# aligirayhanozbay/poisson_CNN

Measured on AMD Instinct MI355X. Metric: grids/sec (fwd+bwd) at 1024^2, higher is better.
Workload: dtype f32; 1 GPU; c4: Homogeneous_Poisson_NN_Legacy(hpnn.json) full train step (fwd+bwd+loss+Adam), 8 x 1024x1024 Dirichlet grids per GPU; global_batch=8, parallelism=dp1, math=fp32, ranks_seen=1

## Files before the change

### include/pcnn.h

```cpp
#ifndef PCNN_H
#define PCNN_H
#include <stddef.h>
#include <stdint.h>
#ifdef __cplusplus
extern "C" {
#endif

typedef struct pcnn_handle_s* pcnn_handle;

enum { PCNN_PAD_CONSTANT = 0, PCNN_PAD_SYMMETRIC = 1, PCNN_PAD_REFLECT = 2 };
enum { PCNN_ACT_LINEAR = 0, PCNN_ACT_LEAKY_RELU = 1, PCNN_ACT_TANH = 2, PCNN_ACT_RELU = 3 };
enum { PCNN_POOL_AVERAGE = 0, PCNN_POOL_MAX = 1 };
enum { PCNN_RESIZE_NEAREST = 0, PCNN_RESIZE_BILINEAR = 1, PCNN_RESIZE_BICUBIC = 2,
       PCNN_RESIZE_BICUBIC_LEGACY_ALIGN_CORNERS = 3  };

int pcnn_create(int device, void* hip_stream, pcnn_handle* out);
int pcnn_destroy(pcnn_handle h);
int pcnn_set_stream(pcnn_handle h, void* hip_stream);
int pcnn_sync(pcnn_handle h);
const char* pcnn_last_error(pcnn_handle h);
int pcnn_version(void);
uint32_t pcnn_crc32c(const void* data, size_t n, uint32_t crc);

#define PCNN_UNIQUE_ID_BYTES 128
// ... 77 lines not shown
int pcnn_conv2d_epilogue_bwd_absmax(pcnn_handle h, int64_t npix, int C, const float* dy, int lddy, const float* a, int lda,
                                    const float* bn_scale, int act, float act_alpha, float* dz, int lddz, float* dbias,
                                    float* dsum_dy_a, float* dsum_dy, float* dz_absmax, void* workspace, size_t workspace_bytes);

int pcnn_pad_fold_bwd(pcnn_handle h, int N, int H, int W, int C, int pt, int pb, int pl, int pr, int pad_mode,
                      const float* gp, int ldgp, float* gx, int ldgx, int accumulate);
int pcnn_pad_fold_bwd_post_eligible(int C, int ldgp, int ld_add, const void* gp, const void* add_to, const pcnn_post_desc* post, int lddz, const void* dz);
int pcnn_pad_fold_bwd_post(pcnn_handle h, int N, int H, int W, int C, int pt, int pb, int pl, int pr, int pad_mode, const float* gp, int ldgp,
                           const float* add_to, int ld_add, const pcnn_post_desc* post, const float* bn_scale, float* dsum_dy_a, float* dsum_dy,
                           float* dz, int lddz, void* workspace, size_t workspace_bytes);

int pcnn_bn_fold(pcnn_handle h, int n, const float* gamma, const float* beta, const float* mean, const float* var, float eps,
                 float* scale, float* shift);
int pcnn_bn_fold_bwd(pcnn_handle h, int n, const float* s_dy_a, const float* s_dy, const float* mean, const float* var, float eps,
                     float* dgamma, float* dbeta);

int pcnn_channel_affine(pcnn_handle h, int64_t npix, int C, const float* x, int ldx, const float* scale, const float* shift,
                        const float* residual, int ld_res, float* y, int ldy);
int pcnn_bn_train_fwd(pcnn_handle h, int64_t npix, int C, const float* a, int lda, const float* gamma, const float* beta, float eps,
                      float momentum, float* moving_mean, float* moving_var, float* mean, float* inv_std, float* scale, float* scratch_2C,
                      const float* residual, int ld_res, float* y, int ldy, void* workspace, size_t workspace_bytes);
int pcnn_bn_train_bwd(pcnn_handle h, int64_t npix, int C, const float* dy, int lddy, const float* a, int lda, const float* scale,
                      const float* mean, const float* inv_std, float* dgamma, float* dbeta, float* scratch_4C, float* da, int ldda,
                      void* workspace, size_t workspace_bytes);

int pcnn_pool2d_fwd(pcnn_handle h, int kind, int N, int H, int W, int C, int f, const float* x, int ldx, float* y, int ldy);
int pcnn_pool2d_bwd(pcnn_handle h, int kind, int N, int H, int W, int C, int f, const float* x, int ldx,
                    const float* y, int ldy, const float* dy, int lddy, float* dx, int lddx, int accumulate);

int pcnn_deconv_fwd(pcnn_handle h, int N, int hc, int wc, int Cin, int H, int W, int Cout, int f, const float* x, int ldx,
                    const float* k, const float* bias, float alpha, float beta, float* y, int ldy);
int pcnn_deconv_bwd_data(pcnn_handle h, int N, int hc, int wc, int Cin, int H, int W, int Cout, int f, const float* dy, int lddy,
                         const float* k, float alpha, float* dx, int lddx);
size_t pcnn_deconv_wgrad_workspace(int N, int hc, int wc, int Cin, int Cout, int f);
int pcnn_deconv_bwd_filter(pcnn_handle h, int N, int hc, int wc, int Cin, int H, int W, int Cout, int f, const float* x, int ldx,
                           const float* dy, int lddy, float alpha, float* dk, float* dbias, void* workspace, size_t workspace_bytes);

typedef struct {
  int N, H, W, Cin, ldx;
  int Ho, Wo, Cout, ldy;
  int k;
  int act; float act_alpha;
  float dropout_rate; uint32_t dropout_seed; uint32_t dropout_layer;
  int ld_act_out;
  int accumulate;
} pcnn_wide_desc;
int pcnn_wide_conv2d_fwd(pcnn_handle h, const pcnn_wide_desc* d, const float* x, const float* w, const float* bias, float* y);
int pcnn_wide_conv2d_dgrad(pcnn_handle h, const pcnn_wide_desc* d, const float* dz, const float* wf, const float* act_out, float* dx);
size_t pcnn_wide_conv2d_wgrad_workspace(const pcnn_wide_desc* d);
int pcnn_wide_conv2d_wgrad(pcnn_handle h, const pcnn_wide_desc* d, const float* x, const float* dz, float* dw, float* dbias, void* workspace,
                           size_t workspace_bytes);
int pcnn_wide_deconv_fwd(pcnn_handle h, const pcnn_wide_desc* d, const float* x, const float* k, const float* bias, float* y);
int pcnn_wide_deconv_bwd_data(pcnn_handle h, const pcnn_wide_desc* d, const float* dz, const float* k, const float* act_out, float* dx);
size_t pcnn_wide_deconv_bwd_filter_workspace(const pcnn_wide_desc* d);
int pcnn_wide_deconv_bwd_filter(pcnn_handle h, const pcnn_wide_desc* d, const float* x, const float* dz, float* dk, void* workspace,
                                size_t workspace_bytes);

int pcnn_resize_tables(int method, int n_in, int n_out, int32_t* idx , float* wt );
int pcnn_resize_fwd(pcnn_handle h, int N, int hc, int wc, int C, int Ho, int Wo, const float* x, int ldx,
                    const int32_t* idx_y, const float* wt_y, const int32_t* idx_x, const float* wt_x,
                    float alpha, float beta, float* y, int ldy);
typedef struct pcnn_resize_src {
  const float* x; int hc, wc, ldx;
  const int32_t* idx_y; const float* wt_y; const int32_t* idx_x; const float* wt_x;
} pcnn_resize_src;
int pcnn_resize_fwd_multi_eligible(int N, int C, int Ho, int Wo, int nsrc, const pcnn_resize_src* src, const float* y, int ldy);
// ... 135 lines not shown
```

### poisson_cnn_amd/csrc/deconv_mfma.hip

```cpp
#include "pcnn_internal.h"

namespace {

struct DeconvParams {
  int N, hc, wc, Cin, H, W, Cout, f, py, px;
  const float* x; int ldx;
  const float* wp;
  const float* bias;
  float alpha, beta;
  float* y; int ldy;
  const float* dy; int lddy;
  float* dx; int lddx;
  float* partial;
  int tiles_x, S;
  float* dummy;
};

__global__ void pack_deconv_fwd_kernel(const float* __restrict__ k, float* __restrict__ wp, int taps, int Cin, int Cout, int ng) {
  const int64_t total = (int64_t)taps * ng * 2 * 32 * 4;
  for (int64_t i = (int64_t)blockIdx.x * blockDim.x + threadIdx.x; i < total; i += (int64_t)gridDim.x * blockDim.x) {
    const int j = i & 3; int64_t r = i >> 2; const int co = r & 31; r >>= 5; const int h = r & 1; r >>= 1; const int g = r % ng; const int tap = r / ng;
    const int ci = 8 * g + 4 * h + j;
    wp[i] = (ci < Cin && co < Cout) ? k[((int64_t)tap * Cout + co) * Cin + ci] : 0.f;
  }
// ... 227 lines not shown
  hipLaunchKernelGGL(pack_deconv_bwd_kernel, dim3((unsigned)std::min<int64_t>(pcnn_cdiv64(tot, 256), 1024)), dim3(256), 0, h->stream, k,
                     static_cast<float*>(h->scratch), f * f, Cin, Cout, ng);
  DeconvParams p{};
  p.N = N; p.hc = hc; p.wc = wc; p.Cin = Cin; p.H = H; p.W = W; p.Cout = Cout; p.f = f; p.py = (hc * f - H) / 2; p.px = (wc * f - W) / 2;
  p.dy = dy; p.lddy = lddy; p.wp = static_cast<const float*>(h->scratch); p.alpha = alpha; p.dx = dx; p.lddx = lddx;
  p.tiles_x = pcnn_cdiv(wc, 32);
  const int64_t groups = (int64_t)N * hc * p.tiles_x;
  hipLaunchKernelGGL(deconv_bwd_data_mfma_kernel, dim3((unsigned)groups), dim3(256), 0, h->stream, p);
  PCNN_CHECK_LAUNCH(h, "pcnn_deconv_bwd_data(mfma)");
  return 0;
}

int pcnn_deconv_bwd_filter_splits(int N, int hc, int f) {
  int S = 1024 / (f * f);
  const int rows4 = (N * hc + 3) / 4;
  if (S > rows4) S = rows4;
  if (S < 1) S = 1;
  if (S > 256) S = 256;
  return S;
}

int pcnn_deconv_bwd_filter_mfma(pcnn_handle h, int N, int hc, int wc, int Cin, int H, int W, int Cout, int f, const float* x, int ldx, const float* dy,
                                int lddy, float* partial, int* S_out) {
  if (Cin > 32 || Cout > 32) return -1;
  DeconvParams p{};
  p.N = N; p.hc = hc; p.wc = wc; p.Cin = Cin; p.H = H; p.W = W; p.Cout = Cout; p.f = f; p.py = (hc * f - H) / 2; p.px = (wc * f - W) / 2;
  p.x = x; p.ldx = ldx; p.dy = dy; p.lddy = lddy; p.partial = partial;
  p.S = pcnn_deconv_bwd_filter_splits(N, hc, f);
  *S_out = p.S;
  hipLaunchKernelGGL(deconv_bwd_filter_mfma_kernel, dim3(p.S, f * f), dim3(256), 0, h->stream, p);
  PCNN_CHECK_LAUNCH(h, "pcnn_deconv_bwd_filter(mfma)");
  return 0;
}
```

### poisson_cnn_amd/layers.py

```python
import numpy as np
import torch

from . import ops
from .utils import advanced_pad_amounts, canonical_activation, glorot_limit, same_pad_amounts, split_indices


class ParamStore:

    def __init__(self):
        self.specs = []
        self.bn_layers = []
        self.finalized = False

    def add(self, name, shape, init, kind='w'):
        assert not self.finalized
        self.specs.append((name, tuple(int(s) for s in shape), init, kind))
        return name

    def add_bn(self, name, c):
        off = sum(ch for _, ch in self.bn_layers)
        self.bn_layers.append((name, c))
        for suffix, init, kind in (('gamma', 'ones', 'bn_gamma'), ('beta', 'zeros', 'bn_beta'), ('moving_mean', 'zeros', 'bn_mean'),
                                   ('moving_variance', 'ones', 'bn_var')):
            self.add('%s/%s' % (name, suffix), (c,), init, kind)
# ... 449 lines not shown
        else:
            ops.pool2d_bwd(self.x, d, self.f, self.pool, dx=d_in, accumulate=True)
        self.x = None
        return ret

    def out_hw(self, H, W):
        return int((H / self.f) * self.up), int((W / self.f) * self.up)


class bottleneck_block_deconvupsample(_bottleneck_base):

    def __init__(self, store, ctx, name, cin, *, deconv_kernel_size, deconv_use_bias=True, **kw):
        super().__init__(store, ctx, name, cin, **kw)
        self.dk = int(deconv_kernel_size)
        self.store = store
        self.ctx = ctx
        self.deconv_use_bias = deconv_use_bias
        store.add(name + '/deconv/kernel', (self.dk, self.dk, self.filters, self.filters), 'glorot')
        if deconv_use_bias:
            store.add(name + '/deconv/bias', (self.filters,), 'glorot')

    def forward_convs(self, x, training=True, pooled=None):
        return self._down_and_convs(x, training, pooled)

    def forward_up(self, o, hw, merged, alpha, beta, training=True):
        self.note_upsampled(o, training)
        self.up_into(o, hw, merged, alpha, beta)

    def up_into(self, o, hw, merged, alpha, beta):
        assert self.out_hw(*hw) == tuple(hw), 'deconv branch must restore the input resolution'
        ops.deconv_fwd(o, self.store.w[self.name + '/deconv/kernel'], self.store.w[self.name + '/deconv/bias'] if self.deconv_use_bias else None,
                       tuple(hw), self.up, alpha=alpha, beta=beta, out=merged)

    def note_upsampled(self, o, training=True):
        self.coarse = o if training else None

    def forward_into(self, x, merged, alpha, beta, training=True, pooled=None):
        self.forward_up(self.forward_convs(x, training, pooled), (x.shape[1], x.shape[2]), merged, alpha, beta, training)

    def backward_up(self, dmerged, alpha):
        g = self.store.g
        k = self.store.w[self.name + '/deconv/kernel']
        o = self.coarse
        self.coarse = None
        ops.deconv_bwd_filter(o, dmerged, self.up, alpha=alpha, dk=g[self.name + '/deconv/kernel'],
                              dbias=g[self.name + '/deconv/bias'] if self.deconv_use_bias else None, ws=self.ctx.ws, kernel_size=(self.dk, self.dk))
        return ops.deconv_bwd_data(dmerged, k, (o.shape[1], o.shape[2]), self.up, alpha=alpha)

    def backward_convs(self, dcoarse, d_in):
        return self._backward_convs_and_down(dcoarse, d_in)

    def backward_from(self, dmerged, alpha, d_in):
        return self.backward_convs(self.backward_up(dmerged, alpha), d_in)


class bottleneck_block_multilinearupsample(_bottleneck_base):

    def __init__(self, store, ctx, name, cin, *, resize_method='bilinear', **kw):
        super().__init__(store, ctx, name, cin, **kw)
        self.method = resize_method.lower()
        if self.method not in ops.RESIZE:
            raise ValueError('unsupported resize method ' + resize_method)

    def forward_convs(self, x, training=True, pooled=None):
        return self._down_and_convs(x, training, pooled)

# ... 200 lines not shown
```

### poisson_cnn_amd/models.py

```python
import copy

import os

import numpy as np
import torch

from . import layers as L
from . import ops
from .utils import get_init_arguments_from_config, split_indices


def process_normalizations(normalizations):
    types, defaults = ['rhs_max_magnitude'], [False]
    if normalizations is None:
        return dict(zip(types, defaults))
    normalizations = dict(normalizations)
    for k, d in zip(types, defaults):
        normalizations.setdefault(k, d)
    if isinstance(normalizations['rhs_max_magnitude'], bool) and normalizations['rhs_max_magnitude']:
        normalizations['rhs_max_magnitude'] = 1.0
    return normalizations


def process_output_scaling_modes(output_scalings):
# ... 233 lines not shown
            logs = {'loss': float('nan'), 'mse': float('nan')}
            step = -1
            if n > 0:
                fetch.request(0)
            for step in range(n):
                inp, tar = fetch.take()
                logs = self.train_step((tuple(inp), tar))
                if step + 1 < n:
                    fetch.request(step + 1)
                logs = _host_logs(logs)
                for k in agg:
                    agg[k] += logs[k]
                for cb in callbacks:
                    cb.on_batch_end(step, logs)
                if self.stop_training:
                    break
            logs = {'loss': logs['loss'], 'mse': logs['mse'], 'lr': self.optimizer.learning_rate,
                    'loss_epoch_mean': agg['loss'] / max(step + 1, 1), 'mse_epoch_mean': agg['mse'] / max(step + 1, 1)}
            for k in history:
                history[k].append(logs[k])
            if verbose:
                print('Epoch %d/%d - loss: %.6g - mse: %.6g - lr: %.3g (epoch mean loss %.6g)'
                      % (epoch + 1, epochs, logs['loss'], logs['mse'], logs['lr'], logs['loss_epoch_mean']), flush=True)
            for cb in callbacks:
                cb.on_epoch_end(epoch, logs)
            if hasattr(dataset, 'on_epoch_end'):
                dataset.on_epoch_end()
            if self.stop_training:
                break
        return history


_BRANCH_STREAMS = os.environ.get('PCNN_BRANCH_STREAMS', '1') != '0'


class Homogeneous_Poisson_NN_Legacy(_ModelBase):
    model_name = 'Homogeneous_Poisson_NN_Legacy'

    def __init__(self, data_format='channels_first', final_convolutions_config=None, pre_bottleneck_convolutions_config=None,
                 bottleneck_deconv_config=None, bottleneck_multilinear_config=None, input_normalization=None, output_scaling=None,
                 use_batchnorm=False, postsmoother_iterations=5, use_scaling=False, use_positional_embeddings=True, scaling_config=None,
                 gradient_accumulation_steps=None, bc_type='dirichlet', device=None, seed=0, batchnorm_training=False):
        if data_format not in ('channels_first', 'channels_last'):
            raise ValueError('data_format must be channels_first or channels_last')
        if pre_bottleneck_convolutions_config is None:
            raise ValueError('Provide a config for pre bottleneck convolutions')
        if bottleneck_deconv_config is None or bottleneck_multilinear_config is None:
            raise ValueError('Provide a config for bottleneck blocks')
        if final_convolutions_config is None:
            raise ValueError('Provide a config for final convolutions')
        if bc_type.lower() not in ('dirichlet', 'neumann'):
            raise ValueError('bc_type can only be neumann or dirichlet.')
        self._init_device(device, _CPU_NOTE_RAISES)
        self.ndims = 2
        self.data_format = data_format
        self.gradient_accumulation_steps = gradient_accumulation_steps
        self.input_normalization = process_normalizations(input_normalization)
        self.output_scaling = process_output_scaling_modes(output_scaling)
        self.use_batchnorm = use_batchnorm
        self.use_positional_embeddings = use_positional_embeddings
        self.neumann = bc_type.lower() == 'neumann'
        self.store = S = L.ParamStore()
        S.bn_training = bool(batchnorm_training)
        self.ctx = C = L.Context()
        C.enable_side_stream()

# ... 85 lines not shown
        for c in self.pre:
            x = c.forward(x, training=training, x_absmax=hint)
            hint = c.out_absmax
        initial = x
        F = self.filters
        cat = ops.empty((N, H, W, 2 * F), self.device)
        merged = cat[..., F:]
        blocks = self.bottleneck_deconv_blocks + self.bottleneck_multilinear_blocks
        alpha = 1.0 / float(len(blocks) * F)
        pyr = self._pool_pyramid(initial, blocks)
        coarse = [b for b in blocks if b.f >= self.COARSE_FACTOR]
        order = [b for b in blocks if b not in coarse] + coarse
        pending = {}
        self._branch_streams = {}
        if coarse and self.ctx.use_side and _BRANCH_STREAMS:
            main = torch.cuda.current_stream()
            ready = torch.cuda.Event()
            ready.record(main)
            for k, b in enumerate(coarse):
                st = self.ctx.branch_stream(k + 1 if b.f in pyr else 0)
                with torch.cuda.stream(st):
                    st.wait_event(ready)
                    o = b.forward_convs(initial, training, pyr[b.f][0] if b.f in pyr else None)
                    done = torch.cuda.Event()
                    done.record(st)
                pending[b] = (o, done)
                if training:
                    self._branch_streams[b] = st
        ntail = 0
        while ntail < min(3, len(order) - 1) and hasattr(order[len(order) - 1 - ntail], 'method'):
            ntail += 1
        if ntail < 2:
            ntail = 0
        tail = []
        for i, b in enumerate(order):
            if b in pending:
                o, done = pending[b]
                torch.cuda.current_stream().wait_event(done)
                o.record_stream(torch.cuda.current_stream())
            else:
                o = b.forward_convs(initial, training, pyr[b.f][0] if b.f in pyr else None)
            b.note_upsampled(o, training)
            if i >= len(order) - ntail:
                tail.append((b, o))
            else:
                b.up_into(o, (H, W), merged, alpha, 0.0 if i == 0 else 1.0)
        if tail:
            beta0 = 0.0 if ntail == len(order) else 1.0
            if ops.resize_fwd_multi([o for _, o in tail], (H, W), [b.method for b, _ in tail], alpha=alpha, beta=beta0, out=merged) is None:
                for k, (b, o) in enumerate(tail):
                    b.up_into(o, (H, W), merged, alpha, beta0 if k == 0 else 1.0)
        self._pyr = pyr if training else None
        self.non_bottleneck_conv.forward(initial, out=cat[..., :F], training=training)
        x = self.post_merge_conv.forward(cat, training=training)
        x = self.post_merge_resnet.forward(x, training=training, x_absmax=self.post_merge_conv.out_absmax)
        d = dense_inp
        for lyr in self.dx_dense_layers:
            d = lyr.forward(d, training=training)
        xs = ops.channel_scale_fwd(x, d)
        if training:
            self._saved = {'initial': initial, 'scale_in': x, 'dx_info': d, 'shape': (N, H, W)}
        x = xs
        hint = None
        for lyr in self.final:
            x = lyr.forward(x, training=training, x_absmax=hint)
            hint = lyr.out_absmax
        if self.scaling is not None:
            x = self.scaling.forward(x, rhs_hw.view(N, H, W, 1), training=training)
        x = ops.bc_ring_fwd(x, self.neumann)
        if self.postsmoother is not None:
            x = self.postsmoother.forward(x, rhs_hw.view(N, H, W, 1), _dx_pair(dx), training=training)
        return x.view(N, 1, H, W)

    def backward(self, dpred):
        sv = self._saved
        self._saved = None
        N, H, W = sv['shape']
# ... 396 lines not shown
```

### poisson_cnn_amd/ops.py

```python
import ctypes
from ctypes import byref, c_float, c_int, c_int64, c_size_t, c_void_p

import numpy as np
import torch

from . import _lib
from ._lib import ConvDesc

PAD_MODES = {'CONSTANT': 0, 'SYMMETRIC': 1, 'REFLECT': 2}
ACTS = {'linear': 0, 'leaky_relu': 1, 'tanh': 2, 'relu': 3}
POOLS = {'average': 0, 'avg': 0, 'max': 1}
RESIZE = {'nearest': 0, 'bilinear': 1, 'bicubic': 2, 'bicubic_legacy': 3}
LEAKY_ALPHA = 0.2
BN_EPS = 1e-3

_handles = {}
MATH_MODES = {'fp32': 0, 'split_f16': 1}
_math_mode = MATH_MODES[__import__('os').environ.get('PCNN_MATH', 'fp32')]


def set_math_mode(mode):
    global _math_mode
    _math_mode = MATH_MODES[mode]
    for h in _handles.values():
# ... 539 lines not shown
def _deconv_same_pads(k, hc, wc, H, W, f):
    kh, kw = k.shape[0], k.shape[1]
    if hc != -(-H // f) or wc != -(-W // f):
        raise ValueError('SAME transposed convolution needs input = ceil(output / stride): got %s for output %s at stride %d' % ((hc, wc), (H, W), f))
    return max((hc - 1) * f + kh - H, 0) // 2, max((wc - 1) * f + kw - W, 0) // 2


def _deconv_general_fwd(x, k, bias, out_hw, f, alpha, beta, out):
    N, hc, wc, Cin = x.shape
    kh, kw, Cout, _ = k.shape
    H, W = out_hw
    pt, pl = _deconv_same_pads(k, hc, wc, H, W, f)
    x_up = subsample_bwd(x, ((hc - 1) * f + 1, (wc - 1) * f + 1), f)
    y = conv2d_fwd(x_up, flip_transpose_weights(k.contiguous()), bias, pad_top=kh - 1 - pt, pad_left=kw - 1 - pl, out_hw=(H, W))
    if out is None:
        return y if alpha == 1.0 else axpby(alpha, y, 0.0, y)
    return axpby(alpha, y, beta, out)


def deconv_fwd(x, k, bias, out_hw, f, *, alpha=1.0, beta=0.0, out=None):
    N, hc, wc, Cin = x.shape
    Cout = k.shape[2]
    H, W = out_hw
    if k.shape[0] != f or k.shape[1] != f:
        return _deconv_general_fwd(x, k, bias, out_hw, f, alpha, beta, out)
    y = out if out is not None else empty((N, H, W, Cout), x.device)
    _launch('deconv_fwd', 2.0 * N * H * W * Cin * Cout,
            lambda: handle().call('pcnn_deconv_fwd', c_int(N), c_int(hc), c_int(wc), c_int(Cin), c_int(H), c_int(W), c_int(Cout), c_int(f), _p(x), c_int(_ld(x)),
                                  _p(k), _p(bias), c_float(alpha), c_float(beta), _p(y), c_int(_ld(y))),
            4.0 * (N * hc * wc * Cin + N * H * W * Cout * (2 if beta != 0.0 else 1) + f * f * Cin * Cout))
    return y


def deconv_bwd_data(dy, k, coarse_hw, f, *, alpha=1.0, out=None):
    N, H, W, Cout = dy.shape
    Cin = k.shape[3]
    hc, wc = coarse_hw
    if k.shape[0] != f or k.shape[1] != f:
        pt, pl = _deconv_same_pads(k, hc, wc, H, W, f)
        full = conv2d_fwd(dy, k.contiguous(), None, pad_top=pt, pad_left=pl, out_hw=((hc - 1) * f + 1, (wc - 1) * f + 1))
        dx_ = subsample(full, f)
        if alpha != 1.0:
            axpby(alpha, dx_, 0.0, dx_)
        if out is None:
            return dx_
        return axpby(1.0, dx_, 0.0, out)
    dx = out if out is not None else empty((N, hc, wc, Cin), dy.device)
    handle().call('pcnn_deconv_bwd_data', c_int(N), c_int(hc), c_int(wc), c_int(Cin), c_int(H), c_int(W), c_int(Cout), c_int(f), _p(dy), c_int(_ld(dy)),
                  _p(k), c_float(alpha), _p(dx), c_int(_ld(dx)))
    return dx


def deconv_bwd_filter(x, dy, f, *, alpha=1.0, dk=None, dbias=None, ws=None, kernel_size=None):
    N, hc, wc, Cin = x.shape
    _, H, W, Cout = dy.shape
    if kernel_size is not None and tuple(kernel_size) != (f, f):
        kh, kw = kernel_size
        pt, pl = max((hc - 1) * f + kh - H, 0) // 2, max((wc - 1) * f + kw - W, 0) // 2
        x_up = subsample_bwd(x, ((hc - 1) * f + 1, (wc - 1) * f + 1), f)
        dwf = conv2d_wgrad(x_up, dy, (kh, kw, Cin, Cout), pad_top=kh - 1 - pt, pad_left=kw - 1 - pl, ws=ws)
        g = flip_transpose_weights(dwf)
        if dk is None:
            dk = g if alpha == 1.0 else axpby_flat(alpha, g, 0.0, g)
        else:
            axpby_flat(alpha, g, 0.0, dk)
        if dbias is not None:
# ... 692 lines not shown
```

### poisson_cnn_amd/csrc/spectral_conv.hip

```cpp
#include "spectral_common.h"
#include <math.h>
#include <stdlib.h>
#include <array>
#include <vector>

int pcnn_spectral_conv_fwd(pcnn_handle h, const pcnn_conv_desc* d, const float* x, const float* w, const float* bias, const float* bn_scale,
                           const float* bn_shift, const float* residual, float* y, float* act_out);
int pcnn_spectral_conv_wgrad(pcnn_handle h, const pcnn_conv_desc* d, const float* x, const float* dz, float* dw);
bool pcnn_spectral_eligible(pcnn_handle h, const pcnn_conv_desc* d, bool wgrad);
bool pcnn_conv_small_fwd_eligible(const pcnn_conv_desc* d);
bool pcnn_conv_fwd_takes_narrow_route(pcnn_handle h, const pcnn_conv_desc* d);

using namespace pcnn_spec;


namespace {

constexpr int T = 32, ROWS = 1024, NSLOT = 512;
constexpr int TAB_G = 0, TAB_GI = 1024, TAB_F2 = 2048, TAB_FI2 = 4096, TAB_GI2 = 6144, TAB_FLOATS = TAB32_FLOATS;
static_assert(TAB_GI2 + 1024 == TAB_FLOATS, "table block");
constexpr size_t LDS_U = (size_t)T * T * 32 * sizeof(float);
constexpr size_t LDS_INV = LDS_U + 1024 * sizeof(float);
__host__ __device__ __forceinline__ int64_t sp_item(int64_t item) { return pcnn_spec::sp_item(item, ROWS); }

// ... 421 lines not shown
#pragma unroll
    for (int u = 0; u < WU; ++u) {
      const bool ok = tb + 2 * u + half < t1;
      const float a0 = ok ? ar[u] : 0.f, a1 = ok ? ai[u] : 0.f;
      acc[0] = mfma(fmaf(-s_cplx, a1, a0), br[u], acc[0]);
      acc[1] = mfma(a0, bi[u] - br[u], acc[1]);
      acc[2] = mfma(a1, fmaf(s_cplx, br[u], bi[u]), acc[2]);
    }
#pragma unroll
    for (int u = 0; u < WU; ++u) { ar[u] = nar[u]; ai[u] = nai[u]; br[u] = nbr[u]; bi[u] = nbi[u]; }
  }
  float* o = p.part + (((int64_t)part * p.nslot + slot) * p.gin + gi) * 4 * 1024 + c;
#pragma unroll
  for (int qd = 0; qd < 3; ++qd) {
    float old[16];
    if (p.accumulate) {
#pragma unroll
      for (int r = 0; r < 16; ++r) old[r] = o[qd * 1024 + acc_row(r, half) * 32];
    }
#pragma unroll
    for (int r = 0; r < 16; ++r) o[qd * 1024 + acc_row(r, half) * 32] = p.accumulate ? old[r] + acc[qd][r] : acc[qd][r];
  }
}

struct MixWParams { const float* zs; const float* xs; float* ys; float* part; const float* wsp; const int4* slots; int ntile, gx, rows, nslot, Cz, cpt, accumulate; };

__global__ __launch_bounds__(256, 2) void spec_mixw_kernel(MixWParams p) {
  const int tid = threadIdx.x, lane = tid & 63, half = lane >> 5, c = lane & 31;
  const int wave = __builtin_amdgcn_readfirstlane(tid >> 6);
  const int slot = blockIdx.x, g = blockIdx.z;
  const int part = blockIdx.y * 4 + wave;
  const int4 sl = p.slots[slot];
  const int rr = sl.x, ri = sl.y;
  float hr[16], hi[16];
  const bool real2 = sl.z == 1;
  const float s_neg = real2 ? 0.f : -1.f, s_pos = real2 ? 0.f : 1.f;
  int kind = sl.z;
  asm volatile("" : "+v"(kind));
  const float s_cplx = kind == 1 ? 0.f : 1.f;
  {
    const int co = c % p.cpt;
#pragma unroll
    for (int j = 0; j < 16; ++j) {
      const int kc = j + 16 * half, ci = kc % p.cpt;
      float wr = 0.f, wi = 0.f;
      if (ci < p.Cz && kc / p.cpt == c / p.cpt) {
        const float* wg = p.wsp + pcnn_spec::sp_item(ci * p.gx + g, p.rows) + co;
        wr = wg[rr * RS]; wi = wg[ri * RS];
      }
      hr[j] = wr; hi[j] = wi;
    }
  }
  const int nMt = (p.ntile + 31) >> 5;
  const int mstride = gridDim.y * 4;
  const float* xr = p.xs + rr * RS, *xi = p.xs + ri * RS;
  const float* dr = p.zs + rr * RS, *di = p.zs + ri * RS;
  const int qi = lane & 3, c4 = c & ~3;
  const bool odd = lane & 1, upper = lane & 2;
  auto load_w = [&](int mt, int b, f32x4 (&w)[4]) {
    const int tt = mt * 32 + 8 * b + 2 * qi + half;
    const unsigned tc = (unsigned)(tt < p.ntile ? tt : 0);
    const unsigned ix = (unsigned)pcnn_spec::sp_item((int64_t)tc * p.gx + g, p.rows) + c4, id = (unsigned)pcnn_spec::sp_item(tc, p.rows) + c4;
    w[0] = __builtin_nontemporal_load(reinterpret_cast<const f32x4*>(&xr[ix])); w[1] = __builtin_nontemporal_load(reinterpret_cast<const f32x4*>(&xi[ix]));
    w[2] = *reinterpret_cast<const f32x4*>(&dr[id]); w[3] = *reinterpret_cast<const f32x4*>(&di[id]);
  };
  f32x16 accp[3] = {zero16(), zero16(), zero16()};
  auto mfma_w = [&](int mt, int b, f32x4 (&w)[4]) {
    float t[4][4];
#pragma unroll
    for (int q = 0; q < 4; ++q) {
#pragma unroll
      for (int j = 0; j < 4; ++j) t[q][j] = w[q][j];
      quad_transpose(t[q][0], t[q][1], t[q][2], t[q][3], odd, upper);
    }
#pragma unroll
    for (int j = 0; j < 4; ++j) {
      const bool ok = mt * 32 + 8 * b + 2 * j + half < p.ntile;
      const float a0 = ok ? t[0][j] : 0.f, a1 = ok ? t[1][j] : 0.f;
      accp[0] = mfma(fmaf(-s_cplx, a1, a0), t[2][j], accp[0]);
      accp[1] = mfma(a0, t[3][j] - t[2][j], accp[1]);
      accp[2] = mfma(a1, fmaf(s_cplx, t[2][j], t[3][j]), accp[2]);
    }
  };
  f32x4 aq[2][2], ws[2][4];
  auto load_a_part = [&](int mt, int pp, int sl2) {
    const int tile = min(mt * 32 + c, p.ntile - 1);
    const float* base = p.zs + pcnn_spec::sp_item(tile, p.rows) + 16 * half + (pp ? ri : rr) * RS + 8 * sl2;
    aq[sl2][0] = *reinterpret_cast<const f32x4*>(base);
    aq[sl2][1] = *reinterpret_cast<const f32x4*>(base + 4);
  };
  int mt = part;
  if (mt < nMt) {
    load_w(mt, 0, ws[0]); load_w(mt, 1, ws[1]);
    load_a_part(mt, 0, 0); load_a_part(mt, 0, 1);
  }
  auto m_tile = [&](int mt) {
    const int mn = mt + mstride < nMt ? mt + mstride : mt;
    f32x16 acc[2] = {zero16(), zero16()};
    auto mix_quarter = [&](int qu) {
#pragma unroll
      for (int e = 0; e < 8; ++e) {
        const int j = 8 * (qu & 1) + e;
        const float av = aq[qu & 1][e >> 2][e & 3];
        if (qu < 2) {
          acc[0] = mfma(av, hr[j], acc[0]);
          acc[1] = mfma(av * s_neg, hi[j], acc[1]);
        } else {
          acc[0] = mfma(av * s_pos, hi[j], acc[0]);
          acc[1] = mfma(av, real2 ? hi[j] : hr[j], acc[1]);
        }
      }
    };
    mfma_w(mt, 0, ws[0]); load_w(mt, 2, ws[0]);     __builtin_amdgcn_sched_barrier(0);
    mix_quarter(0);       load_a_part(mt, 1, 0);    __builtin_amdgcn_sched_barrier(0);
    mfma_w(mt, 1, ws[1]); load_w(mt, 3, ws[1]);     __builtin_amdgcn_sched_barrier(0);
    mix_quarter(1);       load_a_part(mt, 1, 1);    __builtin_amdgcn_sched_barrier(0);
    mfma_w(mt, 2, ws[0]); load_w(mn, 0, ws[0]);     __builtin_amdgcn_sched_barrier(0);
    mix_quarter(2);       load_a_part(mn, 0, 0);    __builtin_amdgcn_sched_barrier(0);
    mfma_w(mt, 3, ws[1]); load_w(mn, 1, ws[1]);     __builtin_amdgcn_sched_barrier(0);
    mix_quarter(3);       load_a_part(mn, 0, 1);    __builtin_amdgcn_sched_barrier(0);
#pragma unroll
    for (int nt = 0; nt < 2; ++nt) {
      const int row = nt ? ri : rr;
#pragma unroll
      for (int r = 0; r < 16; ++r) {
        const int trow = mt * 32 + acc_row(r, half);
        p.ys[pcnn_spec::sp_item((int64_t)trow * p.gx + g, p.rows) + row * RS + c] = acc[nt][r];
      }
    }
  };
  if (mt < nMt) {
    m_tile(mt);
    for (mt += mstride; mt < nMt; mt += mstride) m_tile(mt);
  }
  float* o = p.part + (((int64_t)part * p.nslot + slot) * p.gx + g) * 4 * 1024 + c;
#pragma unroll
  for (int qd = 0; qd < 3; ++qd) {
    float old[16];
    if (p.accumulate) {
#pragma unroll
      for (int r = 0; r < 16; ++r) old[r] = o[qd * 1024 + acc_row(r, half) * 32];
    }
#pragma unroll
    for (int r = 0; r < 16; ++r) o[qd * 1024 + acc_row(r, half) * 32] = p.accumulate ? old[r] + accp[qd][r] : accp[qd][r];
  }
}

__global__ __launch_bounds__(256) void spec_wcombine_kernel(const float* __restrict__ part, const int4* __restrict__ slots, float* __restrict__ csp, int S, int gin, int Cin, float isign, int cpt, int rows) {
  const int nslot = rows / 2;
  const int slot = blockIdx.x, gi = blockIdx.y;
  const int4 sl = slots[slot];
  for (int e = threadIdx.x; e < 1024; e += 256) {
    const int cil = e >> 5, co = e & 31, ci = gi * 32 + cil;
    if (ci >= Cin || cil >= cpt || co >= cpt) continue;
    float P[3] = {0.f, 0.f, 0.f};
    for (int s = 0; s < S; ++s)
      for (int sub = 0; sub < 32 / cpt; ++sub) {
        const float* b = part + (((int64_t)s * nslot + slot) * gin + gi) * 4 * 1024 + (sub * cpt + cil) * 32 + sub * cpt + co;
#pragma unroll
        for (int qd = 0; qd < 3; ++qd) P[qd] += b[qd * 1024];
      }
// ... 568 lines not shown
```

Before: 43.10 grids/s.

## Fuse multiple branch deconv upsamplings into one multi-source MFMA kernel

Adds a multi-branch transposed-convolution forward kernel. For each output row segment it accumulates every eligible branch's upsampled contribution in LDS and writes the merged result to global memory once, in place of one deconv launch per branch that each reads and rewrites the merged tensor. The model routes the leading run of branches whose kernel size equals the upsample factor through this path and falls back to per-branch calls when the inputs are not eligible. The new kernel needs 64KB+ of LDS per block, repacks each branch's filters on every call, and may lose per-branch kernel specialisation.

Measured after the change: 43.22 grids/s (median of 5 runs). No clear change (+0.3%).

```diff
diff --git a/include/pcnn.h b/include/pcnn.h
--- a/include/pcnn.h
+++ b/include/pcnn.h
@@ -133,6 +133,12 @@
                     const float* k, const float* bias, float alpha, float beta, float* y, int ldy);
 int pcnn_deconv_bwd_data(pcnn_handle h, int N, int hc, int wc, int Cin, int H, int W, int Cout, int f, const float* dy, int lddy,
                          const float* k, float alpha, float* dx, int lddx);
+typedef struct pcnn_deconv_src {
+  const float* x; int hc, wc, ldx, Cin, f;
+  const float* k; const float* bias; float alpha;
+} pcnn_deconv_src;
+int pcnn_deconv_fwd_multi_eligible(int N, int H, int W, int Cout, int nsrc, const pcnn_deconv_src* src, const float* y, int ldy);
+int pcnn_deconv_fwd_multi(pcnn_handle h, int N, int H, int W, int Cout, int nsrc, const pcnn_deconv_src* src, float* y, int ldy);
 size_t pcnn_deconv_wgrad_workspace(int N, int hc, int wc, int Cin, int Cout, int f);
 int pcnn_deconv_bwd_filter(pcnn_handle h, int N, int hc, int wc, int Cin, int H, int W, int Cout, int f, const float* x, int ldx,
                            const float* dy, int lddy, float alpha, float* dk, float* dbias, void* workspace, size_t workspace_bytes);
diff --git a/poisson_cnn_amd/csrc/deconv_mfma.hip b/poisson_cnn_amd/csrc/deconv_mfma.hip
--- a/poisson_cnn_amd/csrc/deconv_mfma.hip
+++ b/poisson_cnn_amd/csrc/deconv_mfma.hip
@@ -283,3 +283,133 @@
   PCNN_CHECK_LAUNCH(h, "pcnn_deconv_bwd_filter(mfma)");
   return 0;
 }
+
+constexpr int DM_L = 512;
+constexpr int DM_MAX_BRANCHES = 8;
+constexpr int DM_LDS_FLOATS = DM_L * 32 + 256;
+
+namespace {
+
+struct DeconvMultiBranch {
+  const float* x; const float* wp; const float* bias;
+  int hc, wc, ldx, Cin, f, py, px;
+  float alpha;
+};
+struct DeconvMultiParams {
+  int N, H, W, Cout, nb, bx;
+  float* y; int ldy;
+  DeconvMultiBranch b[DM_MAX_BRANCHES];
+};
+
+__global__ __launch_bounds__(256) void deconv_fwd_multi_kernel(DeconvMultiParams p) {
+  extern __shared__ float dm_row[];
+  const int lane = threadIdx.x & 63, half = lane >> 5, col = lane & 31;
+  const int wave = __builtin_amdgcn_readfirstlane(threadIdx.x >> 6);
+  int bid = blockIdx.x;
+  const int Xb = (bid % p.bx) * DM_L; bid /= p.bx;
+  const int Y = bid % p.H, n = bid / p.H;
+  const int Xe = min(Xb + DM_L, p.W);
+  const int dmy = DM_L * 32 + threadIdx.x;
+  for (int bi = 0; bi < p.nb; ++bi) {
+    const DeconvMultiBranch& br = p.b[bi];
+    const int f = br.f, ng = (br.Cin + 7) >> 3;
+    const int ty = (Y + br.py) % f, yc = (Y + br.py) / f;
+    const int xc_lo = (Xb + br.px) / f, xc_hi = (Xe - 1 + br.px) / f;
+    const int units = ((xc_hi - xc_lo) / 32 + 1) * f;
+    const float bias = (br.bias && col < p.Cout) ? br.bias[col] : 0.f;
+    const f32x4* wl = reinterpret_cast<const f32x4*>(br.wp) + half * 32 + col;
+    const float* xrow = br.x + ((int64_t)n * br.hc + yc) * br.wc * br.ldx;
+    auto load_ab = [&](int u, f32x4 (&a)[4], f32x4 (&b)[4]) {
+      const int xc_l = xc_lo + 32 * (u / f) + col;
+      const bool pv = xc_l < br.wc;
+      const float* xsrc = xrow + (int64_t)(pv ? xc_l : br.wc - 1) * br.ldx;
+      const int tp = ty * f + u % f;
+#pragma unroll
+      for (int g = 0; g < 4; ++g) {
+        const int ch = 8 * g + 4 * half;
+        const f32x4 v = *reinterpret_cast<const f32x4*>(xsrc + min(ch, br.Cin - 4));
+        const bool use = pv && ch < br.Cin;
+#pragma unroll
+        for (int j = 0; j < 4; ++j) a[g][j] = use ? v[j] : 0.f;
+        b[g] = wl[(int64_t)(tp * ng + min(g, ng - 1)) * 64];
+      }
+    };
+    f32x4 a0[4], b0[4], a1[4], b1[4];
+    if (wave < units) load_ab(wave, a0, b0);
+    for (int u = wave; u < units; u += 4) {
+      load_ab(min(u + 4, units - 1), a1, b1);
+      f32x16 acc;
+#pragma unroll
+      for (int i = 0; i < 16; ++i) acc[i] = 0.f;
+#pragma unroll
+      for (int g = 0; g < 4; ++g)
+#pragma unroll
+        for (int j = 0; j < 4; ++j) acc = __builtin_amdgcn_mfma_f32_32x32x2f32(a0[g][j], b0[g][j], acc, 0, 0, 0);
+      const int x0 = xc_lo + 32 * (u / f), tx = u % f;
+      int at[16];
+#pragma unroll
+      for (int i = 0; i < 16; ++i) {
+        const int xc = x0 + 8 * (i >> 2) + 4 * half + (i & 3);
+        const int X = xc * f + tx - br.px;
+        const bool ok = col < p.Cout && xc < br.wc && X >= Xb && X < Xe;
+        at[i] = ok ? (X - Xb) * 32 + col : dmy;
+      }
+      if (bi == 0) {
+#pragma unroll
+        for (int i = 0; i < 16; ++i) dm_row[at[i]] = br.alpha * (acc[i] + bias);
+      } else {
+        float old[16];
+#pragma unroll
+        for (int i = 0; i < 16; ++i) old[i] = dm_row[at[i]];
+#pragma unroll
+        for (int i = 0; i < 16; ++i) dm_row[at[i]] = old[i] + br.alpha * (acc[i] + bias);
+      }
+#pragma unroll
+      for (int g = 0; g < 4; ++g) { a0[g] = a1[g]; b0[g] = b1[g]; }
+    }
+    __syncthreads();
+  }
+  float* yrow = p.y + (((int64_t)n * p.H + Y) * p.W + Xb) * p.ldy;
+  for (int idx = threadIdx.x; idx < (Xe - Xb) * 8; idx += 256) {
+    const int pix = idx >> 3, q = idx & 7;
+    if (4 * q < p.Cout) *reinterpret_cast<f32x4*>(yrow + (int64_t)pix * p.ldy + 4 * q) = *reinterpret_cast<const f32x4*>(dm_row + pix * 32 + 4 * q);
+  }
+}
+
+}
+
+extern "C" int pcnn_deconv_fwd_multi_eligible(int N, int H, int W, int Cout, int nsrc, const pcnn_deconv_src* src, const float* y, int ldy) {
+  if (!src || !y || nsrc < 1 || nsrc > DM_MAX_BRANCHES || N < 1 || H < 1 || W < 1) return 0;
+  if (Cout < 4 || Cout > 32 || Cout % 4 != 0 || ldy < Cout || ldy % 4 != 0 || !aligned16(y)) return 0;
+  if ((int64_t)N * H * pcnn_cdiv(W, DM_L) > 0x7fffffff) return 0;
+  for (int k = 0; k < nsrc; ++k) {
+    const pcnn_deconv_src& s = src[k];
+    if (!s.x || !s.k || s.f < 1 || s.Cin < 4 || s.Cin > 32 || s.Cin % 4 != 0 || s.ldx < s.Cin || s.ldx % 4 != 0 || !aligned16(s.x)) return 0;
+    if (s.hc != pcnn_cdiv(H, s.f) || s.wc != pcnn_cdiv(W, s.f)) return 0;
+  }
+  return 1;
+}
+
+extern "C" int pcnn_deconv_fwd_multi(pcnn_handle h, int N, int H, int W, int Cout, int nsrc, const pcnn_deconv_src* src, float* y, int ldy) {
+  PCNN_REQUIRE(h, h && pcnn_deconv_fwd_multi_eligible(N, H, W, Cout, nsrc, src, y, ldy), "pcnn_deconv_fwd_multi: not eligible (ask pcnn_deconv_fwd_multi_eligible first)");
+  size_t off[DM_MAX_BRANCHES + 1] = {0};
+  for (int k = 0; k < nsrc; ++k)
+    off[k + 1] = off[k] + (((size_t)src[k].f * src[k].f * ((src[k].Cin + 7) >> 3) * 64 * 4 * sizeof(float) + 255) & ~(size_t)255);
+  if (!ensure_scratch(h, off[nsrc])) PCNN_FAIL(h, "pcnn_deconv_fwd_multi: cannot allocate filter scratch");
+  DeconvMultiParams p{};
+  p.N = N; p.H = H; p.W = W; p.Cout = Cout; p.nb = nsrc; p.bx = pcnn_cdiv(W, DM_L); p.y = y; p.ldy = ldy;
+  for (int k = 0; k < nsrc; ++k) {
+    const pcnn_deconv_src& s = src[k];
+    const int ng = (s.Cin + 7) >> 3;
+    float* wp = reinterpret_cast<float*>(static_cast<char*>(h->scratch) + off[k]);
+    const int64_t tot = (int64_t)s.f * s.f * ng * 64 * 4;
+    hipLaunchKernelGGL(pack_deconv_fwd_kernel, dim3((unsigned)std::min<int64_t>(pcnn_cdiv64(tot, 256), 1024)), dim3(256), 0, h->stream, s.k, wp, s.f * s.f, s.Cin, Cout, ng);
+    p.b[k] = DeconvMultiBranch{s.x, wp, s.bias, s.hc, s.wc, s.ldx, s.Cin, s.f, (s.hc * s.f - H) / 2, (s.wc * s.f - W) / 2, s.alpha};
+  }
+  const size_t lds = DM_LDS_FLOATS * sizeof(float);
+  if (hipFuncSetAttribute(reinterpret_cast<const void*>(deconv_fwd_multi_kernel), hipFuncAttributeMaxDynamicSharedMemorySize, (int)lds) != hipSuccess)
+    PCNN_FAIL(h, "pcnn_deconv_fwd_multi: cannot reserve %zu B of LDS", lds);
+  hipLaunchKernelGGL(deconv_fwd_multi_kernel, dim3((unsigned)((int64_t)N * H * p.bx)), dim3(256), lds, h->stream, p);
+  PCNN_CHECK_LAUNCH(h, "pcnn_deconv_fwd_multi");
+  return 0;
+}
diff --git a/poisson_cnn_amd/layers.py b/poisson_cnn_amd/layers.py
--- a/poisson_cnn_amd/layers.py
+++ b/poisson_cnn_amd/layers.py
@@ -505,6 +505,13 @@
         ops.deconv_fwd(o, self.store.w[self.name + '/deconv/kernel'], self.store.w[self.name + '/deconv/bias'] if self.deconv_use_bias else None,
                        tuple(hw), self.up, alpha=alpha, beta=beta, out=merged)
 
+    @property
+    def multi_ok(self):
+        return self.dk == self.up
+
+    def up_args(self):
+        return self.store.w[self.name + '/deconv/kernel'], self.store.w[self.name + '/deconv/bias'] if self.deconv_use_bias else None
+
     def note_upsampled(self, o, training=True):
         self.coarse = o if training else None
 
diff --git a/poisson_cnn_amd/models.py b/poisson_cnn_amd/models.py
--- a/poisson_cnn_amd/models.py
+++ b/poisson_cnn_amd/models.py
@@ -289,6 +289,7 @@
 
 
 _BRANCH_STREAMS = os.environ.get('PCNN_BRANCH_STREAMS', '1') != '0'
+_DECONV_MULTI = os.environ.get('PCNN_DECONV_MULTI', '1') != '0'
 
 
 class Homogeneous_Poisson_NN_Legacy(_ModelBase):
@@ -440,7 +441,13 @@
             ntail += 1
         if ntail < 2:
             ntail = 0
-        tail = []
+        nhead = 0
+        if _DECONV_MULTI:
+            while nhead < len(order) - ntail and getattr(order[nhead], 'multi_ok', False):
+                nhead += 1
+            if nhead < 2:
+                nhead = 0
+        tail, head = [], []
         for i, b in enumerate(order):
             if b in pending:
                 o, done = pending[b]
@@ -451,6 +458,14 @@
             b.note_upsampled(o, training)
             if i >= len(order) - ntail:
                 tail.append((b, o))
+            elif i < nhead:
+                head.append((b, o))
+                if i == nhead - 1:
+                    args = [b_.up_args() for b_, _ in head]
+                    if ops.deconv_fwd_multi([o_ for _, o_ in head], [a[0] for a in args], [a[1] for a in args], (H, W), [b_.up for b_, _ in head],
+                                            alphas=[alpha] * nhead, out=merged) is None:
+                        for k, (b_, o_) in enumerate(head):
+                            b_.up_into(o_, (H, W), merged, alpha, 0.0 if k == 0 else 1.0)
             else:
                 b.up_into(o, (H, W), merged, alpha, 0.0 if i == 0 else 1.0)
         if tail:
diff --git a/poisson_cnn_amd/ops.py b/poisson_cnn_amd/ops.py
--- a/poisson_cnn_amd/ops.py
+++ b/poisson_cnn_amd/ops.py
@@ -595,6 +595,32 @@
     return y
 
 
+class DeconvSrc(ctypes.Structure):
+    _fields_ = [('x', c_void_p), ('hc', c_int), ('wc', c_int), ('ldx', c_int), ('Cin', c_int), ('f', c_int), ('k', c_void_p), ('bias', c_void_p), ('alpha', c_float)]
+
+
+def deconv_fwd_multi(xs, ks, biases, out_hw, fs, *, alphas, out):
+    if not 1 <= len(xs) <= 8:
+        return None
+    N, H, W, Cout = out.shape
+    if (H, W) != tuple(out_hw):
+        return None
+    arr = (DeconvSrc * len(xs))()
+    flops, nbytes = 0.0, 4.0 * N * H * W * Cout
+    for i, (x, k, b, f, a) in enumerate(zip(xs, ks, biases, fs, alphas)):
+        if x.dim() != 4 or x.shape[0] != N or k.shape[0] != f or k.shape[1] != f or k.shape[2] != Cout or k.shape[3] != x.shape[3] or not k.is_contiguous():
+            return None
+        arr[i] = DeconvSrc(x.data_ptr(), x.shape[1], x.shape[2], _ld(x), x.shape[3], f, k.data_ptr(), b.data_ptr() if b is not None else None, a)
+        flops += 2.0 * N * H * W * x.shape[3] * Cout
+        nbytes += 4.0 * (x.numel() + k.numel())
+    lib = _lib.load()
+    if not lib.pcnn_deconv_fwd_multi_eligible(c_int(N), c_int(H), c_int(W), c_int(Cout), c_int(len(xs)), arr, _p(out), c_int(_ld(out))):
+        return None
+    _launch('deconv_fwd', flops, lambda: handle().call('pcnn_deconv_fwd_multi', c_int(N), c_int(H), c_int(W), c_int(Cout), c_int(len(xs)), arr, _p(out), c_int(_ld(out))),
+            nbytes)
+    return out
+
+
 def deconv_bwd_data(dy, k, coarse_hw, f, *, alpha=1.0, out=None):
     N, H, W, Cout = dy.shape
     Cin = k.shape[3]
```

## Use 3-mult complex mixing with LDS-staged weights in mixw kernel

Applied to the files above, without the earlier changes.

Replaces the 4-MFMA-per-element complex mixing in spec_mixw_kernel with a Gauss/Karatsuba-style 3-product form. Precomputed combined weights (wr, -wi-wr, wi-wr) are staged in LDS and streamed through a small register window, replacing the 32 per-lane weight registers. Both real and imaginary input rows are loaded together per half, and the outputs are recombined at store time. This cuts MFMA count and register pressure in exchange for LDS traffic, a block barrier, a third accumulator and a different load schedule.

New measurement: 43.35 grids/s before, 43.62 grids/s after, median of 6. No clear change (+0.6%).

```diff
diff --git a/poisson_cnn_amd/csrc/spectral_conv.hip b/poisson_cnn_amd/csrc/spectral_conv.hip
--- a/poisson_cnn_amd/csrc/spectral_conv.hip
+++ b/poisson_cnn_amd/csrc/spectral_conv.hip
@@ -477,25 +477,38 @@
   const int part = blockIdx.y * 4 + wave;
   const int4 sl = p.slots[slot];
   const int rr = sl.x, ri = sl.y;
-  float hr[16], hi[16];
+  __shared__ float fl[48 * 64];
   const bool real2 = sl.z == 1;
-  const float s_neg = real2 ? 0.f : -1.f, s_pos = real2 ? 0.f : 1.f;
   int kind = sl.z;
   asm volatile("" : "+v"(kind));
   const float s_cplx = kind == 1 ? 0.f : 1.f;
   {
     const int co = c % p.cpt;
-#pragma unroll
-    for (int j = 0; j < 16; ++j) {
+    const int wv = tid >> 6;
+#pragma unroll
+    for (int jj = 0; jj < 4; ++jj) {
+      const int j = 4 * wv + jj;
       const int kc = j + 16 * half, ci = kc % p.cpt;
       float wr = 0.f, wi = 0.f;
       if (ci < p.Cz && kc / p.cpt == c / p.cpt) {
         const float* wg = p.wsp + pcnn_spec::sp_item(ci * p.gx + g, p.rows) + co;
         wr = wg[rr * RS]; wi = wg[ri * RS];
       }
-      hr[j] = wr; hi[j] = wi;
-    }
-  }
+      fl[(3 * j) * 64 + lane] = wr;
+      fl[(3 * j + 1) * 64 + lane] = real2 ? wi : -wi - wr;
+      fl[(3 * j + 2) * 64 + lane] = real2 ? 0.f : wi - wr;
+    }
+  }
+  __syncthreads();
+  constexpr int MIXW_WIN = 4;
+  float fw[MIXW_WIN][3];
+  const float* flane = fl + lane;
+  auto fill = [&](int s) {
+#pragma unroll
+    for (int v = 0; v < 3; ++v) fw[s % MIXW_WIN][v] = flane[(3 * (s & 15) + v) * 64];
+  };
+#pragma unroll
+  for (int s = 0; s < MIXW_WIN; ++s) fill(s);
   const int nMt = (p.ntile + 31) >> 5;
   const int mstride = gridDim.y * 4;
   const float* xr = p.xs + rr * RS, *xi = p.xs + ri * RS;
@@ -527,51 +540,46 @@
       accp[2] = mfma(a1, fmaf(s_cplx, t[2][j], t[3][j]), accp[2]);
     }
   };
-  f32x4 aq[2][2], ws[2][4];
-  auto load_a_part = [&](int mt, int pp, int sl2) {
+  f32x4 aq[2][2][2], ws[2][4];
+  auto load_a_part = [&](int mt, int hf) {
     const int tile = min(mt * 32 + c, p.ntile - 1);
-    const float* base = p.zs + pcnn_spec::sp_item(tile, p.rows) + 16 * half + (pp ? ri : rr) * RS + 8 * sl2;
-    aq[sl2][0] = *reinterpret_cast<const f32x4*>(base);
-    aq[sl2][1] = *reinterpret_cast<const f32x4*>(base + 4);
+    const float* base = p.zs + pcnn_spec::sp_item(tile, p.rows) + 16 * half + 8 * hf;
+    aq[hf][0][0] = *reinterpret_cast<const f32x4*>(base + rr * RS); aq[hf][0][1] = *reinterpret_cast<const f32x4*>(base + rr * RS + 4);
+    aq[hf][1][0] = *reinterpret_cast<const f32x4*>(base + ri * RS); aq[hf][1][1] = *reinterpret_cast<const f32x4*>(base + ri * RS + 4);
   };
   int mt = part;
   if (mt < nMt) {
     load_w(mt, 0, ws[0]); load_w(mt, 1, ws[1]);
-    load_a_part(mt, 0, 0); load_a_part(mt, 0, 1);
+    load_a_part(mt, 0); load_a_part(mt, 1);
   }
   auto m_tile = [&](int mt) {
     const int mn = mt + mstride < nMt ? mt + mstride : mt;
-    f32x16 acc[2] = {zero16(), zero16()};
+    f32x16 acc[3] = {zero16(), zero16(), zero16()};
     auto mix_quarter = [&](int qu) {
 #pragma unroll
-      for (int e = 0; e < 8; ++e) {
-        const int j = 8 * (qu & 1) + e;
-        const float av = aq[qu & 1][e >> 2][e & 3];
-        if (qu < 2) {
-          acc[0] = mfma(av, hr[j], acc[0]);
-          acc[1] = mfma(av * s_neg, hi[j], acc[1]);
-        } else {
-          acc[0] = mfma(av * s_pos, hi[j], acc[0]);
-          acc[1] = mfma(av, real2 ? hi[j] : hr[j], acc[1]);
-        }
+      for (int e = 0; e < 4; ++e) {
+        const int st = 4 * qu + e;
+        const float dr_ = aq[qu >> 1][0][qu & 1][e], di_ = aq[qu >> 1][1][qu & 1][e];
+        acc[0] = mfma(fmaf(s_cplx, di_, dr_), fw[st % MIXW_WIN][0], acc[0]);
+        acc[1] = mfma(kind == 1 ? di_ : dr_, fw[st % MIXW_WIN][1], acc[1]);
+        acc[2] = mfma(di_, fw[st % MIXW_WIN][2], acc[2]);
+        fill(st + MIXW_WIN);
       }
     };
     mfma_w(mt, 0, ws[0]); load_w(mt, 2, ws[0]);     __builtin_amdgcn_sched_barrier(0);
-    mix_quarter(0);       load_a_part(mt, 1, 0);    __builtin_amdgcn_sched_barrier(0);
+    mix_quarter(0);                                 __builtin_amdgcn_sched_barrier(0);
     mfma_w(mt, 1, ws[1]); load_w(mt, 3, ws[1]);     __builtin_amdgcn_sched_barrier(0);
-    mix_quarter(1);       load_a_part(mt, 1, 1);    __builtin_amdgcn_sched_barrier(0);
+    mix_quarter(1);       load_a_part(mn, 0);       __builtin_amdgcn_sched_barrier(0);
     mfma_w(mt, 2, ws[0]); load_w(mn, 0, ws[0]);     __builtin_amdgcn_sched_barrier(0);
-    mix_quarter(2);       load_a_part(mn, 0, 0);    __builtin_amdgcn_sched_barrier(0);
+    mix_quarter(2);                                 __builtin_amdgcn_sched_barrier(0);
     mfma_w(mt, 3, ws[1]); load_w(mn, 1, ws[1]);     __builtin_amdgcn_sched_barrier(0);
-    mix_quarter(3);       load_a_part(mn, 0, 1);    __builtin_amdgcn_sched_barrier(0);
-#pragma unroll
-    for (int nt = 0; nt < 2; ++nt) {
-      const int row = nt ? ri : rr;
-#pragma unroll
-      for (int r = 0; r < 16; ++r) {
-        const int trow = mt * 32 + acc_row(r, half);
-        p.ys[pcnn_spec::sp_item((int64_t)trow * p.gx + g, p.rows) + row * RS + c] = acc[nt][r];
-      }
+    mix_quarter(3);       load_a_part(mn, 1);       __builtin_amdgcn_sched_barrier(0);
+#pragma unroll
+    for (int r = 0; r < 16; ++r) {
+      const int trow = mt * 32 + acc_row(r, half);
+      float* o = &p.ys[pcnn_spec::sp_item((int64_t)trow * p.gx + g, p.rows) + c];
+      o[rr * RS] = acc[0][r] + acc[2][r];
+      o[ri * RS] = fmaf(s_cplx, acc[0][r], acc[1][r]);
     }
   };
   if (mt < nMt) {
```
